# zmoon/crt1d

Hardware: AMD Instinct MI355X
Metric: (column x band) solves/sec at 60 layers (higher is better)
Workload: dtype f64

## Files before the change

### crt1d_amd/csrc/api.hip

```cpp
#include <math.h>

#include <algorithm>
#include <type_traits>

#include "crt_internal.hpp"

namespace crt {
namespace {

typedef double d2 __attribute__((ext_vector_type(2)));
constexpr int MAXG = 4;
constexpr int BS_CH = 8;

template <typename TIO>
struct EpiArgsT {
  int ncol, nb, nz, ngroup;
  long long col_stride;
  const double* psi;
  const double* lai;
  const int32_t* g_kind;
  const double* g_param;
  const double* g_at_psi;
  const TIO* leaf_r;
  const TIO* leaf_t;
// ... 1120 lines not shown
  if (scheme != CRT_SCHEME_BL && !bands->soil_r) return CRT_ERR_BAD_ARG;
  if (bands->col_stride != 0 && bands->col_stride < nb) return CRT_ERR_BAD_ARG;
  if (!integ && (!out->I_dr || !out->I_df_d || !out->I_df_u || !out->F)) return CRT_ERR_BAD_ARG;
  const bool tri = scheme == CRT_SCHEME_N79 || scheme == CRT_SCHEME_ZQ;
  const int nextra = scheme == CRT_SCHEME_N79 ? 2 : (scheme == CRT_SCHEME_ZQ || scheme == CRT_SCHEME_G77 || scheme == CRT_SCHEME_BF) ? 3 : 0;
  if (!integ) {
    if (nextra >= 1 && !out->x0) return CRT_ERR_BAD_ARG;
    if (nextra >= 2 && !out->x1) return CRT_ERR_BAD_ARG;
    if (nextra >= 3 && !out->x2) return CRT_ERR_BAD_ARG;
  }
  if (nz < 2) return CRT_ERR_SHAPE;
  if (scheme == CRT_SCHEME_N79 && nz < 3) return CRT_ERR_SHAPE;
  double mu_s = 0.501;
  int method = CRT_TAU_D_QUAD, flags = 0;
  int tune[CRT_NTUNE] = {};
  if (opts) {
    mu_s = opts->mu_s;
    method = opts->tau_d_method;
    flags = opts->flags;
    for (int i = 0; i < CRT_NTUNE; ++i) tune[i] = opts->tune[i];
  }
  {
    static const struct { int key, lo, hi; } range[] = {
        {0, 0, 160 * 1024}, {1, 0, 64}, {2, 0, 255}, {3, 0, 12}, {4, 0, 32}, {8, 0, 16}, {9, 0, 12}, {10, 0, 7}, {11, 0, 12}, {12, 0, 1024}, {13, 0, 3}, {5, 0, 2}, {6, 0, 4}};
    bool known[CRT_NTUNE] = {};
    for (const auto& r : range) {
      known[r.key] = true;
      if (tune[r.key] < r.lo || tune[r.key] > r.hi) return CRT_ERR_BAD_ARG;
    }
    if (tune[8] != 0 && tune[8] != 8 && tune[8] != 12 && tune[8] != 16) return CRT_ERR_BAD_ARG;
    if (tune[9] != 0 && tune[9] != 4 && tune[9] != 8 && tune[9] != 12) return CRT_ERR_BAD_ARG;
    for (int i = 0; i < CRT_NTUNE; ++i)
      if (!known[i] && tune[i] != 0) return CRT_ERR_BAD_ARG;
  }
  if (scheme == CRT_SCHEME_4S && !(mu_s > 0.0 && mu_s < 1.0)) return CRT_ERR_BAD_ARG;
  if (method != CRT_TAU_D_QUAD && method != CRT_TAU_D_9SKY) return CRT_ERR_BAD_ARG;
  const size_t need = crt_hip_workspace_bytes_nb(scheme, ncol, nz, nb);
  if (!workspace || workspace_bytes < need) return CRT_ERR_WORKSPACE;

  hipStream_t s = static_cast<hipStream_t>(stream);
  ColArgs ca;
  ca.ncol = ncol;
  ca.nz = nz;
  ca.scheme = scheme;
  ca.tau_d_method = method;
  ca.mu_s = mu_s;
  ca.psi = cols->psi;
  ca.lai = cols->lai;
  ca.mla = cols->mla;
  ca.g_kind = cols->g_kind;
  ca.g_param = cols->g_param;
  ca.g_at_psi = cols->g_at_psi;
  ca.g_table = cols->g_table;
  ca.ws = static_cast<double*>(workspace);
  if (!(flags & CRT_FLAG_SKIP_PRECOMPUTE)) {
    int st = launch_colpre(ca, s);
    if (st != CRT_OK) return st;
  }
  if (flags & CRT_FLAG_PRECOMPUTE_ONLY) return CRT_OK;

  SolveArgs sa;
  sa.ncol = ncol;
  sa.nb = nb;
  sa.nz = nz;
  sa.reclen = rec_len(scheme, nz);
  sa.col_stride = bands->col_stride;
  sa.ws = static_cast<const double*>(workspace);
  sa.I_dr0 = bands->I_dr0;
  sa.I_df0 = bands->I_df0;
  sa.leaf_r = bands->leaf_r;
  sa.leaf_t = bands->leaf_t;
  sa.soil_r = bands->soil_r;
  sa.o[0] = out->I_dr;
  sa.o[1] = out->I_df_d;
  sa.o[2] = out->I_df_u;
  sa.o[3] = out->F;
  sa.o[4] = out->x0;
  sa.o[5] = out->x1;
  sa.o[6] = out->x2;
  sa.mu_s = mu_s;
  sa.f32 = f32;
  for (int i = 0; i < CRT_NTUNE; ++i) sa.tune[i] = tune[i];
  if (integ) {
    if (scheme == CRT_SCHEME_ZQ_PA) return launch_zqpa_int(sa, *integ, s);
    return tri ? launch_tridiag_int(scheme, sa, *integ, s) : launch_closed_int(scheme, sa, *integ, s);
  }
  if (scheme == CRT_SCHEME_ZQ_PA)
    return launch_zqpa(sa, static_cast<double*>(workspace) + (size_t)ncol * sa.reclen, s);
  const int force = (flags & CRT_FLAG_DIRECT_STORES) ? 1 : 0;
  return tri ? launch_tridiag(scheme, sa, s, force) : launch_closed(scheme, sa, s, force);
}


int crt_hip_solve_f64(int scheme, const crt_columns* cols, const crt_bands* bands, const crt_options* opts,
                      const crt_outputs* out, void* workspace, size_t workspace_bytes, crt_stream_t stream) {
  return solve_impl(scheme, cols, bands, opts, out, workspace, workspace_bytes, stream, 0);
}

int crt_hip_solve_f32(int scheme, const crt_columns* cols, const crt_bands_f32* bands, const crt_options* opts,
                      const crt_outputs_f32* out, void* workspace, size_t workspace_bytes, crt_stream_t stream) {
  static_assert(sizeof(crt_bands_f32) == sizeof(crt_bands) && sizeof(crt_outputs_f32) == sizeof(crt_outputs), "layout");
  return solve_impl(scheme, cols, reinterpret_cast<const crt_bands*>(bands), opts, reinterpret_cast<const crt_outputs*>(out), workspace,
                    workspace_bytes, stream, 1);
}

#define CRT_ENTRY(name, id)                                                                                        \
  int name(const crt_columns* c, const crt_bands* b, const crt_options* o, const crt_outputs* out, void* ws,       \
           size_t wsb, crt_stream_t s) {                                                                           \
    return crt_hip_solve_f64(id, c, b, o, out, ws, wsb, s);                                                        \
  }
CRT_ENTRY(crt_hip_2s_f64, CRT_SCHEME_2S)
CRT_ENTRY(crt_hip_4s_f64, CRT_SCHEME_4S)
CRT_ENTRY(crt_hip_n79_f64, CRT_SCHEME_N79)
// ... 187 lines not shown
```

### crt1d_amd/csrc/colpre.hip

```cpp
#include <math.h>

#include <mutex>

#include "crt_internal.hpp"

namespace crt {

namespace {

constexpr int NQT = CRT_NQ_TAU;
constexpr int NQG = CRT_NQ_G4;
constexpr int NPAN = 6;
constexpr int NGL = 16;
constexpr double PAN_EDGE[NPAN + 1] = {0.0, 1e-4, 1e-3, 1e-2, 0.1, 0.6, 1.0};
static_assert(NPAN * NGL == NQT, "tau_d rule size");
static_assert(2 * NGL == NQG, "4s rule size");

struct QuadConst {
  double psi[NQT], cs[NQT], sn[NQT];
  double w[NQT];
  double w2sc[NQT];
  double gx[NGL], gw[NGL];
  double cs9[CRT_NQ_9SKY], sn9[CRT_NQ_9SKY], sc9[CRT_NQ_9SKY];
};

__constant__ QuadConst qc;
QuadConst h_qc;
std::once_flag h_once;
bool dev_inited[64] = {};
std::mutex dev_mu;

void gauss_legendre(int n, double* x, double* w) {
  for (int i = 0; i < n; ++i) {
    double z = cos(M_PI * (i + 0.75) / (n + 0.5));
    double pp = 0;
    for (int it = 0; it < 100; ++it) {
      double p1 = 1.0, p2 = 0.0;
      for (int j = 1; j <= n; ++j) {
        double p3 = p2;
        p2 = p1;
        p1 = ((2.0 * j - 1.0) * z * p2 - (j - 1.0) * p3) / j;
      }
      pp = n * (z * p1 - p2) / (z * z - 1.0);
      double dz = p1 / pp;
      z -= dz;
      if (fabs(dz) < 1e-16) break;
    }
    x[n - 1 - i] = z;
    w[n - 1 - i] = 2.0 / ((1.0 - z * z) * pp * pp);
// ... 40 lines not shown
constexpr int K0_BLOCK = 128;
constexpr int BL_UNIF_MAX_NZ = 512;
constexpr int BL_CHUNK = 16;
static_assert(K0_BLOCK == 8 * BL_CHUNK && CRT_NQ_TAU % 8 == 0, "bl chunk reduction layout");

__device__ inline double tau_d_quad(const double* kq, double L) {
  double s = 0.0;
  for (int q = 0; q < NQT; ++q) s += qc.w2sc[q] * fexp(-kq[q] * L);
  return s;
}

__device__ inline double one_minus_tau_d_quad(const double* kq, double L) {
  double s = 0.0;
  for (int q = 0; q < NQT; ++q) s -= qc.w2sc[q] * fexpm1(-kq[q] * L);
  return s;
}

__device__ inline double tau_d_9sky(const double* k9, double L) {
  double s = 0.0;
  for (int i = 0; i < CRT_NQ_9SKY; ++i) s += fexp(-k9[i] * L) * qc.sc9[i];
  return s * (2.0 * 0.17453292519943295);
}

__device__ inline double wave_sum64(double v) {
#pragma unroll
  for (int off = 32; off > 0; off >>= 1) v += __shfl_down(v, off, 64);
  return __shfl(v, 0, 64);
}

__global__ __launch_bounds__(K0_BLOCK) void k_colpre(ColArgs a) {
  __shared__ double kq[NQT];
  __shared__ double pmb[NQT];
  __shared__ double pg[NQG];
  __shared__ double k9[CRT_NQ_9SKY];
  __shared__ double sh_kb, sh_dlm, sh_dl, sh_tdu;
  __shared__ int sh_unif;
  __shared__ double xis[104];
  extern __shared__ double bl_lds[];
  double* bl_terms = bl_lds;
  double* bl_gsum = bl_terms + NQT * (BL_CHUNK + 1);
  double* bl_td = bl_gsum + 8 * BL_CHUNK;

  const int c = blockIdx.x;
  const int tid = threadIdx.x, lane = tid & 63, wave = tid >> 6;
  const int nz = a.nz;
  const int kind = a.g_kind[c];
  const double param = a.g_param ? a.g_param[c] : 0.0;
  const double* tab = (kind == CRT_G_TABLE) ? a.g_table + (long long)c * CRT_NQ : nullptr;
  const double* lai = a.lai + (long long)c * nz;
  const int reclen = rec_len(a.scheme, nz);
  double* rec = a.ws + (long long)c * reclen;

  const double gden = tab ? 0.0 : G_den(kind, param);
  for (int q = tid; q < NQT; q += K0_BLOCK) {
    const double g = tab ? tab[q] : G_eval(kind, param, gden, qc.cs[q], qc.sn[q]);
    kq[q] = g / qc.cs[q];
    pmb[q] = qc.w[q] * qc.cs[q] * qc.sn[q] / g;
  }
  if (a.scheme == CRT_SCHEME_4S && tid < NQG) {
    const int iv = tid / NGL, i = tid % NGL;
    double lo, hi;
    g4_interval(a.mu_s, iv, lo, hi);
    const double p = lo + (qc.gx[i] + 1.0) * (hi - lo) / 2;
    const double g = tab ? tab[NQT + tid] : G_eval(kind, param, gden, cos(p), sin(p));
    pg[tid] = qc.gw[i] * (hi - lo) / 2 * g * sin(p);
  }
  if (tid < CRT_NQ_9SKY) {
    const double g = tab ? tab[NQT + NQG + tid] : G_eval(kind, param, gden, qc.cs9[tid], qc.sn9[tid]);
    k9[tid] = g / qc.cs9[tid];
  }
  __syncthreads();

  if (wave == 0) {
    const double psi = a.psi[c];
    const double cs = cos(psi), sn = sin(psi);
    const double G = tab ? a.g_at_psi[c] : G_eval(kind, param, gden, cs, sn);
    const double Kb = G / cs;
    const double dl = (lai[0] - lai[nz - 1]) / (nz - 1);
    const double tol = 4.0 * 2.220446049250313e-16 * fabs(lai[0]);
    bool ok = dl > 0.0;
    double dsum = 0.0;
    double dcnt = 0.0;
    for (int j = lane; j + 1 < nz; j += 64) {
      const double d = lai[j] - lai[j + 1];
      ok = ok && fabs(d - dl) <= tol;
      if (d != 0.0) {
        dsum -= d;
        dcnt += 1.0;
      }
    }
    const bool unif = __all(ok);
    double mubar = 0.0, g1 = 0.0, g2 = 0.0, dlm = 0.0;
    if (a.scheme == CRT_SCHEME_2S) mubar = wave_sum64(pmb[lane] + (lane < NQT - 64 ? pmb[64 + lane] : 0.0));
    if (a.scheme == CRT_SCHEME_4S) {
      g1 = wave_sum64(lane < NGL ? pg[lane] : 0.0);
      g2 = wave_sum64(lane < NGL ? pg[NGL + lane] : 0.0);
    }
    if (a.scheme == CRT_SCHEME_ZQ) dlm = fabs(wave_sum64(dsum) / wave_sum64(dcnt));
    if (lane == 0) {
      rec[S_KB] = Kb;
      rec[S_MU] = cs;
      rec[S_G] = G;
      rec[S_MUBAR] = mubar;
      rec[S_GINT1] = g1;
      rec[S_GINT2] = g2;
      rec[S_DLM] = dlm;
      rec[S_TAUI] = 0.0;
      rec[S_TPSI] = a.scheme == CRT_SCHEME_ZQ ? fexp(-Kb * dlm) : 0.0;
      double cos2 = 0.0;
      if (a.scheme == CRT_SCHEME_2S) {
        const double cm = cos(a.mla[c] * (M_PI / 180.0));
        cos2 = cm * cm;
      }
      rec[S_COS2] = cos2;
      rec[S_LT] = lai[0];
      rec[S_INVMU] = 1.0 / cs;
      rec[S_UNIF] = unif ? 1.0 : 0.0;
      rec[S_DL] = dl;
      rec[S_M] = (double)zqpa_M(nz);
      rec[15] = 0.0;
      sh_kb = Kb;
      sh_dlm = dlm;
      sh_dl = dl;
      sh_unif = unif ? 1 : 0;
    }
  }
  __syncthreads();
  const double Kb = sh_kb;
  if (a.scheme == CRT_SCHEME_ZQ_PA) {
    const int M = zqpa_M(nz);
    const double Lm = lai[0] / M;
    for (int q = tid; q < NQT; q += K0_BLOCK) pmb[q] = qc.w2sc[q] * fexp(-kq[q] * Lm);
    __syncthreads();
    if (wave == 0) {
      const double t = wave_sum64(pmb[lane] + (lane < NQT - 64 ? pmb[64 + lane] : 0.0));
      if (lane == 0) {
        rec[S_TAUI] = t;
        rec[S_TPSI] = fexp(-Kb * Lm);
        double sacc = 0.0;
        xis[0] = 0.0;
        for (int i = 1; i <= M; ++i) {
          sacc += Lm;
          xis[i] = sacc;
        }
      }
    }
    __syncthreads();
// ... 38 lines not shown
          P *= E;
        }
      }
      __syncthreads();
      {
        const int jj = tid & (BL_CHUNK - 1), g = tid / BL_CHUNK;
        double acc = 0.0;
        for (int q = g * (NQT / 8); q < (g + 1) * (NQT / 8); ++q) acc += bl_terms[q * (BL_CHUNK + 1) + jj];
        bl_gsum[g * BL_CHUNK + jj] = acc;
      }
      __syncthreads();
      if (tid < BL_CHUNK && jtop - tid >= 0) {
        double t = 0.0;
#pragma unroll
        for (int g = 0; g < 8; ++g) t += bl_gsum[g * BL_CHUNK + tid];
        bl_td[jtop - tid] = t;
      }
      __syncthreads();
    }
  }
  double* v = rec + REC_HDR;
  for (int j = tid; j < nz; j += K0_BLOCK) {
    const double L = lai[j];
    const double ekl = fexp(-Kb * L);
    switch (a.scheme) {
      case CRT_SCHEME_ZQ:
        v[j] = ekl;
        break;
      case CRT_SCHEME_ZQ_PA: {
        const int M = zqpa_M(nz);
        auto xi = [&](int i) { return xis[i]; };
        v[j] = (j < M) ? fexp(-Kb * xi(M - j)) : 0.0;
        v[nz + j] = ekl;
        int lo = 0;
        for (int i = 1; i < M; ++i)
          if (xi(i) <= L) lo = i;
        const double x0 = xi(lo), x1 = xi(lo + 1);
        double w = (L - x0) / (x1 - x0);
        if (L >= x1) w = 1.0;
        v[2 * nz + j] = (double)(M - lo);
        v[3 * nz + j] = w;
        break;
      }
      case CRT_SCHEME_BL:
        v[j] = L;
        v[nz + j] = ekl;
        v[2 * nz + j] = blu ? bl_td[j] : tau_d_quad(kq, L);
// ... 53 lines not shown
  return hipGetLastError() == hipSuccess ? CRT_OK : CRT_ERR_LAUNCH;
}

void host_quad_nodes(double mu_s, double* psi_nodes) {
  std::call_once(h_once, build_host_tables);
  for (int q = 0; q < NQT; ++q) psi_nodes[q] = h_qc.psi[q];
  for (int t = 0; t < NQG; ++t) {
    double lo, hi;
    g4_interval(mu_s, t / NGL, lo, hi);
    psi_nodes[NQT + t] = lo + (h_qc.gx[t % NGL] + 1.0) * (hi - lo) / 2;
  }
  for (int i = 0; i < CRT_NQ_9SKY; ++i) psi_nodes[NQT + NQG + i] = (5.0 + 10.0 * i) * (M_PI / 180.0);
}

int init_quadrature(hipStream_t s) {
  std::call_once(h_once, build_host_tables);
  int dev = 0;
  if (hipGetDevice(&dev) != hipSuccess) return CRT_ERR_LAUNCH;
  if (dev < 0 || dev >= 64) return CRT_ERR_UNSUPPORTED;
  std::lock_guard<std::mutex> lk(dev_mu);
  if (!dev_inited[dev]) {
    if (hipMemcpyToSymbolAsync(HIP_SYMBOL(qc), &h_qc, sizeof(QuadConst), 0, hipMemcpyHostToDevice, s) != hipSuccess)
      return CRT_ERR_LAUNCH;
    if (hipStreamSynchronize(s) != hipSuccess) return CRT_ERR_LAUNCH;
    dev_inited[dev] = true;
  }
  return CRT_OK;
}

int launch_colpre(const ColArgs& a, hipStream_t s) {
  int st = init_quadrature(s);
  if (st != CRT_OK) return st;
  const size_t dyn = a.scheme == CRT_SCHEME_BL ? (NQT * (BL_CHUNK + 1) + 8 * BL_CHUNK + BL_UNIF_MAX_NZ) * sizeof(double) : 0;
  hipLaunchKernelGGL(k_colpre, dim3(a.ncol), dim3(K0_BLOCK), dyn, s, a);
  return hipGetLastError() == hipSuccess ? CRT_OK : CRT_ERR_LAUNCH;
}

}
```

### crt1d_amd/csrc/crt_internal.hpp

```cpp
#pragma once
#include <hip/hip_runtime.h>
#include <stdint.h>

#include "crt1d_hip.h"

namespace crt {

enum RecScalar {
  S_KB = 0,
  S_MU = 1,
  S_G = 2,
  S_MUBAR = 3,
  S_GINT1 = 4,
  S_GINT2 = 5,
  S_DLM = 6,
  S_TAUI = 7,
  S_TPSI = 8,
  S_COS2 = 9,
  S_LT = 10,
  S_INVMU = 11,
  S_UNIF = 12,
  S_DL = 13,
  S_M = 14,
  REC_HDR = 16
// ... 431 lines not shown
    if constexpr (PROF) ia.aI_dr[o] = adr;
  }
  if (ia.totals) {
    for (int i = threadIdx.x; i < ng * 4; i += blockDim.x) {
      const int g = i >> 2, q = i & 3;
      const int e = q < 2 ? 1 : 0, which = q & 1;
      double t = 0.0;
      for (int r = 0; r < nrow; ++r) t += L.ends[((e * nrow + r) * 2 + which) * INT_MAXG + g];
      ia.totals[((long long)c * ng + g) * 4 + q] = t;
    }
  }
}

__host__ __device__ inline size_t int_lds_doubles(int nz, int nwave, bool rows = false, bool prof = false) {
  const size_t nslot = rows ? (size_t)nwave * 4 : (size_t)nwave;
  return (size_t)nz * nslot * INT_MAXG + 2 * nslot * 2 * INT_MAXG + (size_t)nwave * INT_MAXG +
         (prof ? (size_t)nz * nwave * 2 * INT_MAXG + (size_t)nwave * INT_MAXG : 0);
}

int launch_closed_int(int scheme, const SolveArgs& a, const IntArgs& ia, hipStream_t s);
int launch_tridiag_int(int scheme, const SolveArgs& a, const IntArgs& ia, hipStream_t s);

int launch_colpre(const ColArgs& a, hipStream_t s);
int launch_closed(int scheme, const SolveArgs& a, hipStream_t s, int force);
int launch_tridiag(int scheme, const SolveArgs& a, hipStream_t s, int force);
int init_quadrature(hipStream_t s);
int launch_tau_d(const double* kb_nodes, const double* L, long long n, int method, double* out, hipStream_t s);
int launch_tridiag_tile(int scheme, const SolveArgs& a, hipStream_t s, bool& done);
int launch_tri_tile_n79_f64(const SolveArgs& a, hipStream_t s, bool& done);
int launch_tri_tile_n79_f32(const SolveArgs& a, hipStream_t s, bool& done);
int launch_tri_tile_zq_f64(const SolveArgs& a, hipStream_t s, bool& done);
int launch_tri_tile_zq_f32(const SolveArgs& a, hipStream_t s, bool& done);
int launch_tri_int_n79_f64(const SolveArgs& a, const IntArgs& ia, hipStream_t s);
int launch_tri_int_n79_f32(const SolveArgs& a, const IntArgs& ia, hipStream_t s);
int launch_tri_int_zq_f64(const SolveArgs& a, const IntArgs& ia, hipStream_t s);
int launch_tri_int_zq_f32(const SolveArgs& a, const IntArgs& ia, hipStream_t s);
int launch_zqpa(const SolveArgs& a, double* scratch, hipStream_t s);
int launch_zqpa_int(const SolveArgs& a, const IntArgs& ia, hipStream_t s);
int launch_zqpa_wave(const SolveArgs& g, hipStream_t s);
__host__ __device__ inline int zqpa_M(int nz) { return nz < 100 ? nz : 100; }
void host_quad_nodes(double mu_s, double* psi_nodes);

}
```

### crt1d_amd/csrc/solve_closed.hip

```cpp
#include <algorithm>
#include <type_traits>

#include "crt_internal.hpp"

namespace crt {
namespace {

constexpr double PI = 3.14159265358979323846;

struct BandIn {
  double I_dr0, I_df0, r, t, s;
};

template <int MODE>
__device__ __forceinline__ bool exact_here(bool unif, int j) {
  if constexpr (MODE == 0) return true;
  if constexpr (MODE == 1) return exact_level(j);
  return !unif || exact_level(j);
}

template <typename TIO>
__device__ inline BandIn load_band(const SolveArgs& a, int c, int b, bool need_soil) {
  const long long i = (long long)c * a.col_stride + b;
  BandIn in;
  in.I_dr0 = ldio<TIO>(a.I_dr0, i);
  in.I_df0 = ldio<TIO>(a.I_df0, i);
// ... 519 lines not shown
        } else {
          for (int i = tid; i < nvec; i += nthr) {
            vt v;
#pragma unroll
            for (int w = 0; w < VW; ++w) v[w] = s[mis + VW * i + w];
            gv[i] = v;
          }
        }
        if (tid < mis) g[tid] = s[tid];
        if (tid < tail) g[mis + nvec * VW + tid] = s[mis + nvec * VW + tid];
      }
    }
    }
    if (cfg.flags & 1) __syncthreads(); else lds_barrier();
  }
}

struct PipeTileCfg {
  int ncomp;
  int T;
  int rec_dbl;
};

template <class S, typename TIO, int MAXT, bool FUSED>
__global__ __launch_bounds__(MAXT) void k_pipe(SolveArgs a, PipeTileCfg cfg) {
  constexpr int VW = 16 / (int)sizeof(TIO);
  typedef TIO vt __attribute__((ext_vector_type(VW)));
  extern __shared__ double lds[];
  const int nb = a.nb, nz = a.nz, T = cfg.T;
  const int c = blockIdx.x;
  const int tid = threadIdx.x;
#ifdef CRT_STAMP
  if ((threadIdx.x & 63) == 0) {
    double* dbg = const_cast<double*>(a.ws) + (long long)c * a.reclen + 100 + 3 * (threadIdx.x >> 6);
    dbg[0] = (double)__builtin_amdgcn_s_getreg((31 << 11) | 4);
    dbg[1] = (double)__builtin_amdgcn_s_getreg((31 << 11) | 6);
    dbg[2] = (double)(tid >> 6);
  }
#endif
  BandIn bin = {};
  if (tid < cfg.ncomp) bin = load_band<TIO>(a, c, tid < nb ? tid : 0, S::SOIL);
  {
    const double* src = a.ws + (long long)c * a.reclen;
    for (int i = threadIdx.x; i < a.reclen; i += blockDim.x) lds[i] = src[i];
  }
  __syncthreads();
  const double* rec = lds;
  constexpr int HEAD = FUSED ? 0 : 128 / (int)sizeof(TIO);
  TIO* tile = reinterpret_cast<TIO*>(lds + cfg.rec_dbl) + HEAD;
  const int colrun = HEAD + T * nb, bufrun = S::NARR * colrun;
  if (tid < cfg.ncomp) {
    const bool active = tid < nb;
    const int b = active ? tid : 0;
#ifdef CRT_STAMP
    double* stamp = const_cast<double*>(a.ws) + (long long)c * a.reclen;
    int nstamp = 0;
    const bool stamper = tid == 0;
#define STAMP() do { if (stamper && nstamp < 60) stamp[nstamp++] = (double)wall_clock64(); } while (0)
    STAMP();
#else
#define STAMP() do {} while (0)
#endif
    S st;
    st.init(rec, bin, a);
    STAMP();
// ... 175 lines not shown
        vt x[S::NARR];
#pragma unroll
        for (int k = 0; k < S::NARR; ++k) x[k] = src[k * arrv];
#pragma unroll
        for (int k = 0; k < S::NARR; ++k) __builtin_nontemporal_store(x[k], reinterpret_cast<vt*>(a.o[k]) + go);
        v += dv;
        c += dc;
        if (v >= per) {
          v -= per;
          ++c;
        }
      }
      buf ^= 1;
    }
  }
}

constexpr int MAX_DIRECT_LDS = 64 * 1024;
constexpr int DEFAULT_TILE_LDS = 78 * 1024;
constexpr int MIN_TILE_NB = 4;

int gcd(int x, int y) { return y ? gcd(y, x % y) : x; }

template <class S, typename TIO>
int launch_tile(const SolveArgs& a, hipStream_t s, bool& done) {
  done = false;
  const int nb = a.nb;
  int g_tune[8];
  for (int i = 0; i < 8; ++i) g_tune[i] = a.tune[i];
  if (g_tune[0] <= 0) g_tune[0] = DEFAULT_TILE_LDS;
  const int min_nb = a.tune[12] > 0 ? a.tune[12] : MIN_TILE_NB;
  if (nb < min_nb || nb > 1024) return CRT_OK;
  if ((nb <= 32 || a.tune[5] == 2) && nb <= 128 && a.tune[5] != 1) {
    constexpr int VWp = 16 / (int)sizeof(TIO);
    bool ok = nb % VWp == 0 && (a.nz * nb) % VWp == 0;
    for (int i = 0; i < S::NARR && ok; ++i)
      if (reinterpret_cast<uintptr_t>(a.o[i]) & 15) ok = false;
    if (ok) {
      PackCfg pc;
      pc.ncw = a.tune[6] > 0 ? a.tune[6] : (nb <= 32 ? 1 : 2);
      if (64 * pc.ncw < nb) pc.ncw = (nb + 63) / 64;
      pc.cpw = 64 * pc.ncw / nb;
      const int linep = 128 / (int)sizeof(TIO);
      const int Tap = linep / gcd(nb, linep);
      int Tp = a.tune[4] > 0 ? a.tune[4] : std::max(4, Tap);
      if (Tp > a.nz) Tp = a.nz;
      pc.T = Tp;
      const int cpw = pc.cpw;
      const int nswp = a.tune[3] > 0 ? a.tune[3] : 1;
      const size_t shp = (size_t)((cpw * a.reclen + 1) & ~1) * sizeof(double) + (size_t)2 * cpw * S::NARR * Tp * nb * sizeof(TIO);
      const int thr = 64 * (pc.ncw + nswp);
      if (shp <= 160 * 1024 && thr <= 512 && (Tp * nb) % VWp == 0) {
        auto kern = k_pipe_pack<S, TIO, 512>;
        if (shp > 64 * 1024 &&
            hipFuncSetAttribute(reinterpret_cast<const void*>(kern), hipFuncAttributeMaxDynamicSharedMemorySize, (int)shp) != hipSuccess)
          return (int)CRT_ERR_LAUNCH;
        hipLaunchKernelGGL(kern, dim3((a.ncol + cpw - 1) / cpw), dim3(thr), shp, s, a, pc);
        if (hipGetLastError() != hipSuccess) return (int)CRT_ERR_LAUNCH;
        note_kernel("k_pipe_pack<%s,%s> columns=%d compute_waves=%d T=%d store_waves=%d lds=%zu", S::NAME, sizeof(TIO) == 8 ? "f64" : "f32", pc.cpw,
                    pc.ncw, Tp, nswp, shp);
        done = true;
        return (int)CRT_OK;
      }
    }
  }
  const int CB = nb <= 256 ? 256 / nb : 1;
  const int nthr = CB > 1 ? 256 : ((nb + 63) / 64) * 64;
  const int line = 128 / (int)sizeof(TIO);
  const int Ta = line / gcd(nb, line);
  const size_t per_level = (size_t)S::NARR * CB * nb * sizeof(TIO);
  const size_t target = (size_t)g_tune[0];
  int T = Ta;
  if (per_level * Ta > target) {
    T = (int)(target / per_level);
    if (T < 2) return CRT_OK;
  } else {
    while (per_level * (T + Ta) <= target && T + Ta <= a.nz) T += Ta;
  }
  if (g_tune[1] > 0) T = g_tune[1];
// ... 16 lines not shown
  if (!(g_tune[2] & 4) && (pfused || !(g_tune[2] & 8))) {
    const bool fused = pfused;
    const int pcomp = ((nb + 63) / 64) * 64;
    const size_t plevel = (size_t)S::NARR * nb * sizeof(TIO);
    int nsw = g_tune[3] > 0 ? g_tune[3] : (pcomp <= 64 || (S::HEAVY_INIT && pcomp <= 128 && !fused) ? 1 : pcomp <= 128 ? 2 : 3);
    if (pcomp + 64 * nsw > 1024) nsw = (1024 - pcomp) / 64;
    size_t budget = target;
    if (S::HEAVY_INIT && 2 * plevel * 4 <= 40 * 1024) budget = 40 * 1024;
    if (sizeof(TIO) == 4 && std::is_same<S, Sch2s>::value && 2 * plevel * 4 <= 40 * 1024) budget = 40 * 1024;
    if (!fused && pcomp <= 128 && budget > 32 * 1024) budget = 32 * 1024;
    int Tmax = (int)std::min<size_t>(8, budget / (2 * plevel));
    if (fused && pcomp <= 64 && nb >= 32 && Tmax > 4) Tmax = 4;
    if (Tmax < 4 && 2 * plevel * 4 <= target) Tmax = 4;
    int Tp = Ta <= Tmax ? (Tmax / Ta) * Ta : Tmax;
    if (g_tune[4] > 0) Tp = g_tune[4];
    if (Tp > a.nz) Tp = a.nz;
    PipeTileCfg pc;
    pc.ncomp = pcomp;
    pc.T = Tp;
    pc.rec_dbl = (a.reclen + 1) & ~1;
    const size_t psh = pc.rec_dbl * sizeof(double) + 2 * plevel * Tp + (fused ? 0 : 2 * S::NARR * 128);
    if (nsw >= 1 && Tp >= 2 && psh <= 160 * 1024 && (fused ? (2 * plevel * Ta <= target || g_tune[4] > 0) : true)) {
      const int pthr = pcomp + 64 * nsw;
      auto gop = [&](auto kern) {
        if (psh > 64 * 1024 &&
            hipFuncSetAttribute(reinterpret_cast<const void*>(kern), hipFuncAttributeMaxDynamicSharedMemorySize, (int)psh) != hipSuccess)
          return (int)CRT_ERR_LAUNCH;
        hipLaunchKernelGGL(kern, dim3(a.ncol), dim3(pthr), psh, s, a, pc);
        if (hipGetLastError() != hipSuccess) return (int)CRT_ERR_LAUNCH;
        note_kernel("k_pipe<%s,%s>%s T=%d store_waves=%d lds=%zu", S::NAME, sizeof(TIO) == 8 ? "f64" : "f32", fused ? "" : " generic-flush", Tp, nsw, psh);
        return (int)CRT_OK;
      };
      int st;
      if (fused) st = pthr <= 512 ? gop(k_pipe<S, TIO, 512, true>) : gop(k_pipe<S, TIO, 1024, true>);
      else st = pthr <= 512 ? gop(k_pipe<S, TIO, 512, false>) : gop(k_pipe<S, TIO, 1024, false>);
      done = st == CRT_OK;
      return st;
    }
  }
  auto go = [&](auto kern) {
    if (sh > 64 * 1024 &&
        hipFuncSetAttribute(reinterpret_cast<const void*>(kern), hipFuncAttributeMaxDynamicSharedMemorySize, (int)sh) != hipSuccess)
      return (int)CRT_ERR_LAUNCH;
    hipLaunchKernelGGL(kern, dim3(grid), dim3(nthr), sh, s, a, cfg);
    if (hipGetLastError() != hipSuccess) return (int)CRT_ERR_LAUNCH;
    note_kernel("k_tile<%s,%s>%s CB=%d T=%d lds=%zu", S::NAME, sizeof(TIO) == 8 ? "f64" : "f32", fused ? "" : " generic-flush", CB, T, sh);
    return (int)CRT_OK;
  };
  int st;
  if (fused) {
    if (nthr <= 256) st = go(k_tile<S, TIO, 256, true>);
    else if (nthr <= 512) st = go(k_tile<S, TIO, 512, true>);
    else st = go(k_tile<S, TIO, 1024, true>);
  } else {
    if (nthr <= 256) st = go(k_tile<S, TIO, 256, false>);
    else if (nthr <= 512) st = go(k_tile<S, TIO, 512, false>);
    else st = go(k_tile<S, TIO, 1024, false>);
  }
  done = st == CRT_OK;
  return st;
}

template <class S, typename TIO, int VEC, bool USE_LDS>
int launch_direct_v(const SolveArgs& a, size_t lds_bytes, hipStream_t s) {
  const long long items = (long long)a.ncol * (a.nb / VEC);
  const long long nblk = (items + DBLOCK - 1) / DBLOCK;
  if (nblk > 0x7fffffffLL) return CRT_ERR_UNSUPPORTED;
  hipLaunchKernelGGL((k_direct<S, TIO, VEC, USE_LDS>), dim3((unsigned)nblk), dim3(DBLOCK), USE_LDS ? lds_bytes : 0, s, a);
  if (hipGetLastError() != hipSuccess) return CRT_ERR_LAUNCH;
  note_kernel("k_direct<%s,%s> VEC=%d", S::NAME, sizeof(TIO) == 8 ? "f64" : "f32", VEC);
  return CRT_OK;
}

template <class S, typename TIO>
int launch_scheme(const SolveArgs& a, hipStream_t s, int force) {
  if (force != 1) {
    bool done;
    int st = launch_tile<S, TIO>(a, s, done);
    if (st != CRT_OK || done) return st;
  }
  bool vec2 = (a.nb % 2 == 0) && (a.col_stride % 2 == 0);
  for (int i = 0; i < S::NARR && vec2; ++i)
    if (reinterpret_cast<uintptr_t>(a.o[i]) & (2 * sizeof(TIO) - 1)) vec2 = false;
  const int nbv = a.nb / (vec2 ? 2 : 1);
  const long long cols_per_block = (DBLOCK - 1) / nbv + 2;
  const size_t lds_bytes = (size_t)cols_per_block * a.reclen * sizeof(double);
  const bool use_lds = lds_bytes <= (size_t)MAX_DIRECT_LDS;
  if (vec2)
    return use_lds ? launch_direct_v<S, TIO, 2, true>(a, lds_bytes, s) : launch_direct_v<S, TIO, 2, false>(a, lds_bytes, s);
  return use_lds ? launch_direct_v<S, TIO, 1, true>(a, lds_bytes, s) : launch_direct_v<S, TIO, 1, false>(a, lds_bytes, s);
}

template <class S>
int launch_io(const SolveArgs& a, hipStream_t s, int force) {
  return a.f32 ? launch_scheme<S, float>(a, s, force) : launch_scheme<S, double>(a, s, force);
}

template <class S, typename TIO, int MAXT, bool PROF>
__global__ __launch_bounds__(MAXT) void k_int(SolveArgs a, IntArgs ia, int rec_dbl) {
  extern __shared__ double lds[];
  const int nb = a.nb, nz = a.nz, ng = ia.ngroup;
  const int tid = threadIdx.x, nthr = blockDim.x, lane = tid & 63, wave = tid >> 6, nwave = nthr >> 6;
  const int c = blockIdx.x;
  {
    const double* src = a.ws + (long long)c * a.reclen;
    for (int i = tid; i < a.reclen; i += nthr) lds[i] = src[i];
  }
  __syncthreads();
  const double* rec = lds;
  const IntLds L = int_lds_carve(lds + rec_dbl, nz, nwave, PROF);
  const bool active = tid < nb;
  const int b = active ? tid : 0;
  const BandIn in = load_band<TIO>(a, c, b, S::SOIL);
  S st;
  st.init(rec, in, a);
  double w[INT_MAXG];
#pragma unroll
  for (int g = 0; g < INT_MAXG; ++g) w[g] = (g < ng && active) ? ia.band_w[(long long)g * nb + b] : 0.0;
// ... 40 lines not shown
  if (nthr <= 256) return go(k_int<S, TIO, 256, false>);
  if (nthr <= 512) return go(k_int<S, TIO, 512, false>);
  return go(k_int<S, TIO, 1024, false>);
}

template <class S>
int launch_int_io(const SolveArgs& a, const IntArgs& ia, hipStream_t s) {
  return a.f32 ? launch_int<S, float>(a, ia, s) : launch_int<S, double>(a, ia, s);
}

}

int launch_closed_int(int scheme, const SolveArgs& a, const IntArgs& ia, hipStream_t s) {
  switch (scheme) {
    case CRT_SCHEME_2S: return launch_int_io<Sch2s>(a, ia, s);
    case CRT_SCHEME_4S: return launch_int_io<Sch4s>(a, ia, s);
    case CRT_SCHEME_BL: return launch_int_io<SchBl>(a, ia, s);
    case CRT_SCHEME_G77: return launch_int_io<SchG77<false>>(a, ia, s);
    case CRT_SCHEME_BF: return launch_int_io<SchG77<true>>(a, ia, s);
    default: return CRT_ERR_BAD_ARG;
  }
}

int launch_closed(int scheme, const SolveArgs& a, hipStream_t s, int force) {
  switch (scheme) {
    case CRT_SCHEME_2S: return launch_io<Sch2s>(a, s, force);
    case CRT_SCHEME_4S: return launch_io<Sch4s>(a, s, force);
    case CRT_SCHEME_BL: return launch_io<SchBl>(a, s, force);
    case CRT_SCHEME_G77: return launch_io<SchG77<false>>(a, s, force);
    case CRT_SCHEME_BF: return launch_io<SchG77<true>>(a, s, force);
    default: return CRT_ERR_BAD_ARG;
  }
}

}
```

Before: 3.449 billion.

## Fuse 2S column precompute into the pipelined solve kernel prologue

```diff
diff --git a/crt1d_amd/csrc/api.hip b/crt1d_amd/csrc/api.hip
--- a/crt1d_amd/csrc/api.hip
+++ b/crt1d_amd/csrc/api.hip
@@ -1166,7 +1166,7 @@
   }
   {
     static const struct { int key, lo, hi; } range[] = {
-        {0, 0, 160 * 1024}, {1, 0, 64}, {2, 0, 255}, {3, 0, 12}, {4, 0, 32}, {8, 0, 16}, {9, 0, 12}, {10, 0, 7}, {11, 0, 12}, {12, 0, 1024}, {13, 0, 3}, {5, 0, 2}, {6, 0, 4}};
+        {0, 0, 160 * 1024}, {1, 0, 64}, {2, 0, 255}, {3, 0, 12}, {4, 0, 32}, {8, 0, 16}, {9, 0, 12}, {10, 0, 7}, {11, 0, 12}, {12, 0, 1024}, {13, 0, 3}, {5, 0, 2}, {6, 0, 4}, {15, 0, 1}};
     bool known[CRT_NTUNE] = {};
     for (const auto& r : range) {
       known[r.key] = true;
@@ -1197,7 +1197,12 @@
   ca.g_at_psi = cols->g_at_psi;
   ca.g_table = cols->g_table;
   ca.ws = static_cast<double*>(workspace);
-  if (!(flags & CRT_FLAG_SKIP_PRECOMPUTE)) {
+  const bool k0_in_solve = scheme == CRT_SCHEME_2S && !integ && !(flags & (CRT_FLAG_SKIP_PRECOMPUTE | CRT_FLAG_PRECOMPUTE_ONLY)) &&
+                           tune[15] == 0;
+  if (k0_in_solve) {
+    const int st = init_quadrature(s);
+    if (st != CRT_OK) return st;
+  } else if (!(flags & CRT_FLAG_SKIP_PRECOMPUTE)) {
     int st = launch_colpre(ca, s);
     if (st != CRT_OK) return st;
   }
@@ -1232,7 +1237,7 @@
   if (scheme == CRT_SCHEME_ZQ_PA)
     return launch_zqpa(sa, static_cast<double*>(workspace) + (size_t)ncol * sa.reclen, s);
   const int force = (flags & CRT_FLAG_DIRECT_STORES) ? 1 : 0;
-  return tri ? launch_tridiag(scheme, sa, s, force) : launch_closed(scheme, sa, s, force);
+  return tri ? launch_tridiag(scheme, sa, s, force) : launch_closed(scheme, sa, s, force, k0_in_solve ? &ca : nullptr);
 }
 
 
diff --git a/crt1d_amd/csrc/col_record.hpp b/crt1d_amd/csrc/col_record.hpp
--- /dev/null
+++ b/crt1d_amd/csrc/col_record.hpp
@@ -0,0 +1,169 @@
+#pragma once
+#include <math.h>
+
+#include "crt_internal.hpp"
+
+namespace crt {
+
+constexpr int NQT = CRT_NQ_TAU;
+constexpr int NQG = CRT_NQ_G4;
+constexpr int NGL = 16;
+
+struct QuadConst {
+  double psi[NQT], cs[NQT], sn[NQT];
+  double w[NQT];
+  double w2sc[NQT];
+  double gx[NGL], gw[NGL];
+  double cs9[CRT_NQ_9SKY], sn9[CRT_NQ_9SKY], sc9[CRT_NQ_9SKY];
+};
+
+int upload_quad_closed(const QuadConst& h, hipStream_t s);
+
+namespace {
+
+__constant__ QuadConst qc;
+
+__device__ __forceinline__ double wave_sum64(double v) {
+#pragma unroll
+  for (int off = 32; off > 0; off >>= 1) v += __shfl_down(v, off, 64);
+  return __shfl(v, 0, 64);
+}
+
+struct ColIn {
+  int kind;
+  double param, gden;
+  const double* tab;
+  const double* lai;
+};
+
+__device__ __forceinline__ ColIn col_in(const ColArgs& a, int c) {
+#pragma clang fp contract(off)
+  ColIn in;
+  in.kind = a.g_kind[c];
+  in.param = a.g_param ? a.g_param[c] : 0.0;
+  in.tab = (in.kind == CRT_G_TABLE) ? a.g_table + (long long)c * CRT_NQ : nullptr;
+  in.lai = a.lai + (long long)c * a.nz;
+  in.gden = in.tab ? 0.0 : G_den(in.kind, in.param);
+  return in;
+}
+
+__device__ __forceinline__ void col_node(const ColIn& in, int q, double& kq, double& pmb) {
+#pragma clang fp contract(off)
+  const double g = in.tab ? in.tab[q] : G_eval(in.kind, in.param, in.gden, qc.cs[q], qc.sn[q]);
+  kq = g / qc.cs[q];
+  pmb = qc.w[q] * qc.cs[q] * qc.sn[q] / g;
+}
+
+__device__ __forceinline__ double col_mubar(double t_lo, double t_hi, int lane) {
+#pragma clang fp contract(off)
+  return wave_sum64(t_lo + (lane < NQT - 64 ? t_hi : 0.0));
+}
+
+struct ColSun {
+  double cs, G, Kb;
+};
+
+__device__ __forceinline__ ColSun col_sun(const ColArgs& a, int c, const ColIn& in) {
+#pragma clang fp contract(off)
+  ColSun s;
+  const double psi = a.psi[c];
+  s.cs = cos(psi);
+  const double sn = sin(psi);
+  s.G = in.tab ? a.g_at_psi[c] : G_eval(in.kind, in.param, in.gden, s.cs, sn);
+  s.Kb = s.G / s.cs;
+  return s;
+}
+
+struct ColDl {
+  double dl, dsum, dcnt;
+  bool unif;
+};
+
+__device__ __forceinline__ ColDl col_dl(const ColIn& in, int nz, int lane) {
+#pragma clang fp contract(off)
+  const double* lai = in.lai;
+  const double dl = (lai[0] - lai[nz - 1]) / (nz - 1);
+  const double tol = 4.0 * 2.220446049250313e-16 * fabs(lai[0]);
+  bool ok = dl > 0.0;
+  double dsum = 0.0, dcnt = 0.0;
+  for (int j = lane; j + 1 < nz; j += 64) {
+    const double d = lai[j] - lai[j + 1];
+    ok = ok && fabs(d - dl) <= tol;
+    if (d != 0.0) {
+      dsum -= d;
+      dcnt += 1.0;
+    }
+  }
+  ColDl r;
+  r.dl = dl;
+  r.dsum = dsum;
+  r.dcnt = dcnt;
+  r.unif = __all(ok);
+  return r;
+}
+
+__device__ __forceinline__ double col_cos2(double mla) {
+#pragma clang fp contract(off)
+  const double cm = cos(mla * (M_PI / 180.0));
+  return cm * cm;
+}
+
+__device__ __forceinline__ void col_header(double* rec, const ColSun& s, const ColDl& d, double mubar, double g1, double g2, double dlm, double tpsi,
+                                  double cos2, double lt, int nz) {
+#pragma clang fp contract(off)
+  rec[S_KB] = s.Kb;
+  rec[S_MU] = s.cs;
+  rec[S_G] = s.G;
+  rec[S_MUBAR] = mubar;
+  rec[S_GINT1] = g1;
+  rec[S_GINT2] = g2;
+  rec[S_DLM] = dlm;
+  rec[S_TAUI] = 0.0;
+  rec[S_TPSI] = tpsi;
+  rec[S_COS2] = cos2;
+  rec[S_LT] = lt;
+  rec[S_INVMU] = 1.0 / s.cs;
+  rec[S_UNIF] = d.unif ? 1.0 : 0.0;
+  rec[S_DL] = d.dl;
+  rec[S_M] = (double)zqpa_M(nz);
+  rec[15] = 0.0;
+}
+
+__device__ __forceinline__ double col_ekl(double Kb, double L) {
+#pragma clang fp contract(off)
+  return fexp(-Kb * L);
+}
+
+__device__ __forceinline__ void col_record_2s(const ColArgs& a, int c, double* rec, int tid, int nthr) {
+#pragma clang fp contract(off)
+  const ColIn in = col_in(a, c);
+  const int nz = a.nz;
+  double* ws = a.ws + (long long)c * rec_len(CRT_SCHEME_2S, nz);
+  if (tid < 64) {
+    const int lane = tid;
+    const ColSun sun = col_sun(a, c, in);
+    const ColDl dls = col_dl(in, nz, lane);
+    double kq, t_lo, t_hi = 0.0;
+    col_node(in, lane, kq, t_lo);
+    if (lane < NQT - 64) col_node(in, 64 + lane, kq, t_hi);
+    const double mubar = col_mubar(t_lo, t_hi, lane);
+    if (lane == 0) {
+      const double cos2 = col_cos2(a.mla[c]);
+      col_header(rec, sun, dls, mubar, 0.0, 0.0, 0.0, 0.0, cos2, in.lai[0], nz);
+      col_header(ws, sun, dls, mubar, 0.0, 0.0, 0.0, 0.0, cos2, in.lai[0], nz);
+    }
+  } else if (tid - 64 < nz) {
+    const double Kb = col_sun(a, c, in).Kb;
+    for (int j = tid - 64; j < nz; j += nthr - 64) {
+      const double L = in.lai[j];
+      const double ekl = col_ekl(Kb, L);
+      rec[REC_HDR + j] = L;
+      rec[REC_HDR + nz + j] = ekl;
+      ws[REC_HDR + j] = L;
+      ws[REC_HDR + nz + j] = ekl;
+    }
+  }
+}
+
+}
+}
diff --git a/crt1d_amd/csrc/colpre.hip b/crt1d_amd/csrc/colpre.hip
--- a/crt1d_amd/csrc/colpre.hip
+++ b/crt1d_amd/csrc/colpre.hip
@@ -2,29 +2,17 @@
 
 #include <mutex>
 
-#include "crt_internal.hpp"
+#include "col_record.hpp"
 
 namespace crt {
 
 namespace {
 
-constexpr int NQT = CRT_NQ_TAU;
-constexpr int NQG = CRT_NQ_G4;
 constexpr int NPAN = 6;
-constexpr int NGL = 16;
 constexpr double PAN_EDGE[NPAN + 1] = {0.0, 1e-4, 1e-3, 1e-2, 0.1, 0.6, 1.0};
 static_assert(NPAN * NGL == NQT, "tau_d rule size");
 static_assert(2 * NGL == NQG, "4s rule size");
 
-struct QuadConst {
-  double psi[NQT], cs[NQT], sn[NQT];
-  double w[NQT];
-  double w2sc[NQT];
-  double gx[NGL], gw[NGL];
-  double cs9[CRT_NQ_9SKY], sn9[CRT_NQ_9SKY], sc9[CRT_NQ_9SKY];
-};
-
-__constant__ QuadConst qc;
 QuadConst h_qc;
 std::once_flag h_once;
 bool dev_inited[64] = {};
@@ -111,12 +99,6 @@
   return s * (2.0 * 0.17453292519943295);
 }
 
-__device__ inline double wave_sum64(double v) {
-#pragma unroll
-  for (int off = 32; off > 0; off >>= 1) v += __shfl_down(v, off, 64);
-  return __shfl(v, 0, 64);
-}
-
 __global__ __launch_bounds__(K0_BLOCK) void k_colpre(ColArgs a) {
   __shared__ double kq[NQT];
   __shared__ double pmb[NQT];
@@ -133,19 +115,15 @@
   const int c = blockIdx.x;
   const int tid = threadIdx.x, lane = tid & 63, wave = tid >> 6;
   const int nz = a.nz;
-  const int kind = a.g_kind[c];
-  const double param = a.g_param ? a.g_param[c] : 0.0;
-  const double* tab = (kind == CRT_G_TABLE) ? a.g_table + (long long)c * CRT_NQ : nullptr;
-  const double* lai = a.lai + (long long)c * nz;
+  const ColIn in = col_in(a, c);
+  const int kind = in.kind;
+  const double param = in.param, gden = in.gden;
+  const double* tab = in.tab;
+  const double* lai = in.lai;
   const int reclen = rec_len(a.scheme, nz);
   double* rec = a.ws + (long long)c * reclen;
 
-  const double gden = tab ? 0.0 : G_den(kind, param);
-  for (int q = tid; q < NQT; q += K0_BLOCK) {
-    const double g = tab ? tab[q] : G_eval(kind, param, gden, qc.cs[q], qc.sn[q]);
-    kq[q] = g / qc.cs[q];
-    pmb[q] = qc.w[q] * qc.cs[q] * qc.sn[q] / g;
-  }
+  for (int q = tid; q < NQT; q += K0_BLOCK) col_node(in, q, kq[q], pmb[q]);
   if (a.scheme == CRT_SCHEME_4S && tid < NQG) {
     const int iv = tid / NGL, i = tid % NGL;
     double lo, hi;
@@ -161,57 +139,24 @@
   __syncthreads();
 
   if (wave == 0) {
-    const double psi = a.psi[c];
-    const double cs = cos(psi), sn = sin(psi);
-    const double G = tab ? a.g_at_psi[c] : G_eval(kind, param, gden, cs, sn);
-    const double Kb = G / cs;
-    const double dl = (lai[0] - lai[nz - 1]) / (nz - 1);
-    const double tol = 4.0 * 2.220446049250313e-16 * fabs(lai[0]);
-    bool ok = dl > 0.0;
-    double dsum = 0.0;
-    double dcnt = 0.0;
-    for (int j = lane; j + 1 < nz; j += 64) {
-      const double d = lai[j] - lai[j + 1];
-      ok = ok && fabs(d - dl) <= tol;
-      if (d != 0.0) {
-        dsum -= d;
-        dcnt += 1.0;
-      }
-    }
-    const bool unif = __all(ok);
+    const ColSun sun = col_sun(a, c, in);
+    const ColDl dls = col_dl(in, nz, lane);
+    const double Kb = sun.Kb;
     double mubar = 0.0, g1 = 0.0, g2 = 0.0, dlm = 0.0;
-    if (a.scheme == CRT_SCHEME_2S) mubar = wave_sum64(pmb[lane] + (lane < NQT - 64 ? pmb[64 + lane] : 0.0));
+    if (a.scheme == CRT_SCHEME_2S) mubar = col_mubar(pmb[lane], lane < NQT - 64 ? pmb[64 + lane] : 0.0, lane);
     if (a.scheme == CRT_SCHEME_4S) {
       g1 = wave_sum64(lane < NGL ? pg[lane] : 0.0);
       g2 = wave_sum64(lane < NGL ? pg[NGL + lane] : 0.0);
     }
-    if (a.scheme == CRT_SCHEME_ZQ) dlm = fabs(wave_sum64(dsum) / wave_sum64(dcnt));
+    if (a.scheme == CRT_SCHEME_ZQ) dlm = fabs(wave_sum64(dls.dsum) / wave_sum64(dls.dcnt));
     if (lane == 0) {
-      rec[S_KB] = Kb;
-      rec[S_MU] = cs;
-      rec[S_G] = G;
-      rec[S_MUBAR] = mubar;
-      rec[S_GINT1] = g1;
-      rec[S_GINT2] = g2;
-      rec[S_DLM] = dlm;
-      rec[S_TAUI] = 0.0;
-      rec[S_TPSI] = a.scheme == CRT_SCHEME_ZQ ? fexp(-Kb * dlm) : 0.0;
-      double cos2 = 0.0;
-      if (a.scheme == CRT_SCHEME_2S) {
-        const double cm = cos(a.mla[c] * (M_PI / 180.0));
-        cos2 = cm * cm;
-      }
-      rec[S_COS2] = cos2;
-      rec[S_LT] = lai[0];
-      rec[S_INVMU] = 1.0 / cs;
-      rec[S_UNIF] = unif ? 1.0 : 0.0;
-      rec[S_DL] = dl;
-      rec[S_M] = (double)zqpa_M(nz);
-      rec[15] = 0.0;
+      const double tpsi = a.scheme == CRT_SCHEME_ZQ ? fexp(-Kb * dlm) : 0.0;
+      const double cos2 = a.scheme == CRT_SCHEME_2S ? col_cos2(a.mla[c]) : 0.0;
+      col_header(rec, sun, dls, mubar, g1, g2, dlm, tpsi, cos2, lai[0], nz);
       sh_kb = Kb;
       sh_dlm = dlm;
-      sh_dl = dl;
-      sh_unif = unif ? 1 : 0;
+      sh_dl = dls.dl;
+      sh_unif = dls.unif ? 1 : 0;
     }
   }
   __syncthreads();
@@ -296,7 +241,7 @@
   double* v = rec + REC_HDR;
   for (int j = tid; j < nz; j += K0_BLOCK) {
     const double L = lai[j];
-    const double ekl = fexp(-Kb * L);
+    const double ekl = col_ekl(Kb, L);
     switch (a.scheme) {
       case CRT_SCHEME_ZQ:
         v[j] = ekl;
@@ -396,6 +341,7 @@
   if (!dev_inited[dev]) {
     if (hipMemcpyToSymbolAsync(HIP_SYMBOL(qc), &h_qc, sizeof(QuadConst), 0, hipMemcpyHostToDevice, s) != hipSuccess)
       return CRT_ERR_LAUNCH;
+    if (upload_quad_closed(h_qc, s) != CRT_OK) return CRT_ERR_LAUNCH;
     if (hipStreamSynchronize(s) != hipSuccess) return CRT_ERR_LAUNCH;
     dev_inited[dev] = true;
   }
diff --git a/crt1d_amd/csrc/crt_internal.hpp b/crt1d_amd/csrc/crt_internal.hpp
--- a/crt1d_amd/csrc/crt_internal.hpp
+++ b/crt1d_amd/csrc/crt_internal.hpp
@@ -477,7 +477,7 @@
 int launch_tridiag_int(int scheme, const SolveArgs& a, const IntArgs& ia, hipStream_t s);
 
 int launch_colpre(const ColArgs& a, hipStream_t s);
-int launch_closed(int scheme, const SolveArgs& a, hipStream_t s, int force);
+int launch_closed(int scheme, const SolveArgs& a, hipStream_t s, int force, const ColArgs* k0);
 int launch_tridiag(int scheme, const SolveArgs& a, hipStream_t s, int force);
 int init_quadrature(hipStream_t s);
 int launch_tau_d(const double* kb_nodes, const double* L, long long n, int method, double* out, hipStream_t s);
diff --git a/crt1d_amd/csrc/solve_closed.hip b/crt1d_amd/csrc/solve_closed.hip
--- a/crt1d_amd/csrc/solve_closed.hip
+++ b/crt1d_amd/csrc/solve_closed.hip
@@ -1,7 +1,7 @@
 #include <algorithm>
 #include <type_traits>
 
-#include "crt_internal.hpp"
+#include "col_record.hpp"
 
 namespace crt {
 namespace {
@@ -567,8 +567,9 @@
   int rec_dbl;
 };
 
-template <class S, typename TIO, int MAXT, bool FUSED>
-__global__ __launch_bounds__(MAXT) void k_pipe(SolveArgs a, PipeTileCfg cfg) {
+template <class S, typename TIO, int MAXT, bool FUSED, bool K0 = false>
+__global__ __launch_bounds__(MAXT) void k_pipe(SolveArgs a, PipeTileCfg cfg, ColArgs ca) {
+  static_assert(!K0 || std::is_same<S, Sch2s>::value, "the record prologue forms the 2s record only");
   constexpr int VW = 16 / (int)sizeof(TIO);
   typedef TIO vt __attribute__((ext_vector_type(VW)));
   extern __shared__ double lds[];
@@ -585,7 +586,9 @@
 #endif
   BandIn bin = {};
   if (tid < cfg.ncomp) bin = load_band<TIO>(a, c, tid < nb ? tid : 0, S::SOIL);
-  {
+  if constexpr (K0) {
+    col_record_2s(ca, c, lds, tid, blockDim.x);
+  } else {
     const double* src = a.ws + (long long)c * a.reclen;
     for (int i = threadIdx.x; i < a.reclen; i += blockDim.x) lds[i] = src[i];
   }
@@ -807,8 +810,10 @@
 
 int gcd(int x, int y) { return y ? gcd(y, x % y) : x; }
 
+int k0_before(const ColArgs* k0, hipStream_t s) { return k0 ? launch_colpre(*k0, s) : (int)CRT_OK; }
+
 template <class S, typename TIO>
-int launch_tile(const SolveArgs& a, hipStream_t s, bool& done) {
+int launch_tile(const SolveArgs& a, hipStream_t s, bool& done, const ColArgs* k0) {
   done = false;
   const int nb = a.nb;
   int g_tune[8];
@@ -840,6 +845,7 @@
         if (shp > 64 * 1024 &&
             hipFuncSetAttribute(reinterpret_cast<const void*>(kern), hipFuncAttributeMaxDynamicSharedMemorySize, (int)shp) != hipSuccess)
           return (int)CRT_ERR_LAUNCH;
+        if (const int st = k0_before(k0, s)) return st;
         hipLaunchKernelGGL(kern, dim3((a.ncol + cpw - 1) / cpw), dim3(thr), shp, s, a, pc);
         if (hipGetLastError() != hipSuccess) return (int)CRT_ERR_LAUNCH;
         note_kernel("k_pipe_pack<%s,%s> columns=%d compute_waves=%d T=%d store_waves=%d lds=%zu", S::NAME, sizeof(TIO) == 8 ? "f64" : "f32", pc.cpw,
@@ -902,18 +908,28 @@
     const size_t psh = pc.rec_dbl * sizeof(double) + 2 * plevel * Tp + (fused ? 0 : 2 * S::NARR * 128);
     if (nsw >= 1 && Tp >= 2 && psh <= 160 * 1024 && (fused ? (2 * plevel * Ta <= target || g_tune[4] > 0) : true)) {
       const int pthr = pcomp + 64 * nsw;
+      constexpr bool can_k0 = std::is_same<S, Sch2s>::value;
+      const bool own_k0 = can_k0 && k0 != nullptr;
       auto gop = [&](auto kern) {
         if (psh > 64 * 1024 &&
             hipFuncSetAttribute(reinterpret_cast<const void*>(kern), hipFuncAttributeMaxDynamicSharedMemorySize, (int)psh) != hipSuccess)
           return (int)CRT_ERR_LAUNCH;
-        hipLaunchKernelGGL(kern, dim3(a.ncol), dim3(pthr), psh, s, a, pc);
+        if (!own_k0)
+          if (const int st = k0_before(k0, s)) return st;
+        hipLaunchKernelGGL(kern, dim3(a.ncol), dim3(pthr), psh, s, a, pc, own_k0 ? *k0 : ColArgs{});
         if (hipGetLastError() != hipSuccess) return (int)CRT_ERR_LAUNCH;
-        note_kernel("k_pipe<%s,%s>%s T=%d store_waves=%d lds=%zu", S::NAME, sizeof(TIO) == 8 ? "f64" : "f32", fused ? "" : " generic-flush", Tp, nsw, psh);
+        note_kernel("k_pipe<%s,%s>%s T=%d store_waves=%d lds=%zu%s", S::NAME, sizeof(TIO) == 8 ? "f64" : "f32", fused ? "" : " generic-flush", Tp, nsw, psh,
+                    own_k0 ? " k0=fused" : "");
         return (int)CRT_OK;
       };
       int st;
-      if (fused) st = pthr <= 512 ? gop(k_pipe<S, TIO, 512, true>) : gop(k_pipe<S, TIO, 1024, true>);
-      else st = pthr <= 512 ? gop(k_pipe<S, TIO, 512, false>) : gop(k_pipe<S, TIO, 1024, false>);
+      if (own_k0) {
+        if (fused) st = pthr <= 512 ? gop(k_pipe<S, TIO, 512, true, can_k0>) : gop(k_pipe<S, TIO, 1024, true, can_k0>);
+        else st = pthr <= 512 ? gop(k_pipe<S, TIO, 512, false, can_k0>) : gop(k_pipe<S, TIO, 1024, false, can_k0>);
+      } else {
+        if (fused) st = pthr <= 512 ? gop(k_pipe<S, TIO, 512, true>) : gop(k_pipe<S, TIO, 1024, true>);
+        else st = pthr <= 512 ? gop(k_pipe<S, TIO, 512, false>) : gop(k_pipe<S, TIO, 1024, false>);
+      }
       done = st == CRT_OK;
       return st;
     }
@@ -922,6 +938,7 @@
     if (sh > 64 * 1024 &&
         hipFuncSetAttribute(reinterpret_cast<const void*>(kern), hipFuncAttributeMaxDynamicSharedMemorySize, (int)sh) != hipSuccess)
       return (int)CRT_ERR_LAUNCH;
+    if (const int st = k0_before(k0, s)) return st;
     hipLaunchKernelGGL(kern, dim3(grid), dim3(nthr), sh, s, a, cfg);
     if (hipGetLastError() != hipSuccess) return (int)CRT_ERR_LAUNCH;
     note_kernel("k_tile<%s,%s>%s CB=%d T=%d lds=%zu", S::NAME, sizeof(TIO) == 8 ? "f64" : "f32", fused ? "" : " generic-flush", CB, T, sh);
@@ -953,12 +970,13 @@
 }
 
 template <class S, typename TIO>
-int launch_scheme(const SolveArgs& a, hipStream_t s, int force) {
+int launch_scheme(const SolveArgs& a, hipStream_t s, int force, const ColArgs* k0) {
   if (force != 1) {
     bool done;
-    int st = launch_tile<S, TIO>(a, s, done);
+    int st = launch_tile<S, TIO>(a, s, done, k0);
     if (st != CRT_OK || done) return st;
   }
+  if (const int st = k0_before(k0, s)) return st;
   bool vec2 = (a.nb % 2 == 0) && (a.col_stride % 2 == 0);
   for (int i = 0; i < S::NARR && vec2; ++i)
     if (reinterpret_cast<uintptr_t>(a.o[i]) & (2 * sizeof(TIO) - 1)) vec2 = false;
@@ -972,8 +990,8 @@
 }
 
 template <class S>
-int launch_io(const SolveArgs& a, hipStream_t s, int force) {
-  return a.f32 ? launch_scheme<S, float>(a, s, force) : launch_scheme<S, double>(a, s, force);
+int launch_io(const SolveArgs& a, hipStream_t s, int force, const ColArgs* k0) {
+  return a.f32 ? launch_scheme<S, float>(a, s, force, k0) : launch_scheme<S, double>(a, s, force, k0);
 }
 
 template <class S, typename TIO, int MAXT, bool PROF>
@@ -1060,15 +1078,20 @@
   }
 }
 
-int launch_closed(int scheme, const SolveArgs& a, hipStream_t s, int force) {
+int launch_closed(int scheme, const SolveArgs& a, hipStream_t s, int force, const ColArgs* k0) {
   switch (scheme) {
-    case CRT_SCHEME_2S: return launch_io<Sch2s>(a, s, force);
-    case CRT_SCHEME_4S: return launch_io<Sch4s>(a, s, force);
-    case CRT_SCHEME_BL: return launch_io<SchBl>(a, s, force);
-    case CRT_SCHEME_G77: return launch_io<SchG77<false>>(a, s, force);
-    case CRT_SCHEME_BF: return launch_io<SchG77<true>>(a, s, force);
+    case CRT_SCHEME_2S: return launch_io<Sch2s>(a, s, force, k0);
+    case CRT_SCHEME_4S: return launch_io<Sch4s>(a, s, force, k0);
+    case CRT_SCHEME_BL: return launch_io<SchBl>(a, s, force, k0);
+    case CRT_SCHEME_G77: return launch_io<SchG77<false>>(a, s, force, k0);
+    case CRT_SCHEME_BF: return launch_io<SchG77<true>>(a, s, force, k0);
     default: return CRT_ERR_BAD_ARG;
   }
 }
 
-}
+int upload_quad_closed(const QuadConst& h, hipStream_t s) {
+  return hipMemcpyToSymbolAsync(HIP_SYMBOL(qc), &h, sizeof(QuadConst), 0, hipMemcpyHostToDevice, s) == hipSuccess ? (int)CRT_OK
+                                                                                                                   : (int)CRT_ERR_LAUNCH;
+}
+
+}
```

Result: faster. 3.555 billion, median of 6 (+3.1%).
